# XiYe20/VPTR

Measured on AMD Instinct MI355X. Metric: predicted frames/sec (train step) NAR KTH 10->10 @64x64, higher is better.
Workload: dtype bf16x3 (split-bf16 MFMA, fp32 accumulate/storage); 1 GPU; K64: KTH 64x64x1 10->10, VPTREnc/Dec(528, Tanh, reflect) + VPTRFormerNAR(4 enc + 8 dec, d=528, 8 heads, ws 4, dropout 0.10), single_iter of train_NAR.py, random-init weights; per_gpu_batch=16, global_batch=16, frames_per_clip=10, parallelism=dp1, launch=hipGraph, dec_weight_grads=True, frozen_encoder_convs=winograd F(4x4,3x3), 36 strided-batch P16 products per convolution

## Files before the change

### vptr_amd/csrc/gemm_p16.hip

```cpp
#include "gemm_shared.h"

#include <atomic>

typedef __attribute__((ext_vector_type(4))) short s16x4;
typedef __attribute__((ext_vector_type(8))) short s16x8;

constexpr int P16_STAGE = 40 * 1024;

#define P16_GLDS(laddr, gptr) \
  asm volatile("s_mov_b32 m0, %0\n\tglobal_load_lds_dwordx4 %1, off" ::"s"(__builtin_amdgcn_readfirstlane(laddr)), "v"(gptr) : "memory")

__global__ __launch_bounds__(256) void to_p16_kernel(const float* __restrict__ x, unsigned char* __restrict__ out, int64_t n4) {
  for (int64_t i = (int64_t)blockIdx.x * 256 + threadIdx.x; i < n4; i += (int64_t)gridDim.x * 256) {
    const float4 v = reinterpret_cast<const float4*>(x)[i];
    vptr_p16_store4(out, i * 4, v);
  }
}
extern "C" int vptr_to_p16(const float* x, void* out, int64_t rows, int C, vptr_stream_t stream) {
  VPTR_CHECK(x && out && rows > 0 && C > 0 && C % 16 == 0, "to_p16: C must be a positive multiple of 16 (got %d)", C);
  VPTR_CHECK(((reinterpret_cast<uintptr_t>(x) | reinterpret_cast<uintptr_t>(out)) & 15) == 0, "to_p16: pointers must be 16-byte aligned");
  const int64_t n4 = rows * C / 4;
  to_p16_kernel<<<(unsigned)hmin64((n4 + 255) / 256, 16384), 256, 0, (hipStream_t)stream>>>(x, reinterpret_cast<unsigned char*>(out), n4);
  VPTR_LAUNCH_CHECK();
  return 0;
}

__global__ __launch_bounds__(256) void weight_planes_kernel(const vptr_wplane_entry* __restrict__ tab, const int* __restrict__ tile_start,
                                                            int count) {
  __shared__ float tile[32][33];
  const int b = blockIdx.x;
  int lo = 0, hi = count - 1;
  while (lo < hi) {
    const int mid = (lo + hi + 1) >> 1;
    if (tile_start[mid] <= b) lo = mid;
    else hi = mid - 1;
  }
  const vptr_wplane_entry e = tab[lo];
  const int t = b - tile_start[lo], tk = (e.K + 31) >> 5;
  const int n0 = (t / tk) * 32, k0 = (t % tk) * 32;
  const int r = threadIdx.x >> 3, c = (threadIdx.x & 7) * 4;
  float4 v = make_float4(0.f, 0.f, 0.f, 0.f);
  const bool ok = n0 + r < e.N && k0 + c < e.K;
  if (ok) {
    v = *reinterpret_cast<const float4*>(e.W + (int64_t)(n0 + r) * e.ldw + k0 + c);
    vptr_p16_store4(reinterpret_cast<unsigned char*>(e.Wp), (int64_t)(n0 + r) * e.K + k0 + c, v);
  }
  tile[r][c] = v.x; tile[r][c + 1] = v.y; tile[r][c + 2] = v.z; tile[r][c + 3] = v.w;
  __syncthreads();
  if (k0 + r < e.K && n0 + c < e.N) {
    const float4 w = make_float4(tile[c][r], tile[c + 1][r], tile[c + 2][r], tile[c + 3][r]);
    vptr_p16_store4(reinterpret_cast<unsigned char*>(e.WT), (int64_t)(k0 + r) * e.N + n0 + c, w);
  }
}
extern "C" int vptr_weight_planes(const vptr_wplane_entry* table_dev, const int* tile_start_dev, int count, int total_tiles,
                                  vptr_stream_t stream) {
  VPTR_CHECK(table_dev && tile_start_dev && count > 0 && total_tiles > 0, "weight_planes: bad arguments");
  weight_planes_kernel<<<total_tiles, 256, 0, (hipStream_t)stream>>>(table_dev, tile_start_dev, count);
  VPTR_LAUNCH_CHECK();
  return 0;
}

constexpr int P16_NLOAD = 4;
constexpr int P16_LONE_THREADS = GNT + 64 * P16_NLOAD;
constexpr int p16_vmcnt(const int n) { return 0x0f70 | (n & 15) | ((n >> 4) << 14); }
#define P16_GLDS_NOP(laddr, gptr) \
  asm volatile("s_mov_b32 m0, %0\n\ts_nop 0\n\tglobal_load_lds_dwordx4 %1, off" ::"s"(laddr), "v"(gptr) : "memory")

template <int EPI, int NST>
__global__ __launch_bounds__(NST == 4 ? P16_LONE_THREADS : GNT, NST == 4 ? 3 : 4) void vptr_gemm_p16_kernel(const vptr_gemm_desc p) {
  static_assert(NST == 2 || NST == 4, "two stages (two workgroups per CU) or four (one)");
  constexpr int NFN = 11, BN = 176;
  extern __shared__ __attribute__((aligned(1024))) unsigned char p16_smem[];
  const int tid = threadIdx.x, lane = tid & 63, wave = tid >> 6;
  const int wm = wave & 3, wn = wave >> 2, lr = lane & 15, lq = lane >> 4;
  const int tiles_n = (p.N + BN - 1) / BN;
  const int tiles = tiles_n * ((p.M + GBM - 1) / GBM);
  const int lg = xcd_logical_block();
  const int grp = lg / tiles, tile = lg - grp * tiles;
  const Member mb = member_of(p, p.batch > 1 ? grp : 0);
  const int m0 = (tile / tiles_n) * GBM, n0 = (tile % tiles_n) * BN;
  const int nk = (p.K + 31) >> 5;
  const bool ktail = (p.K & 16) != 0;
  const int nseg = p.ksegs > 1 ? p.ksegs : 1;
  const int64_t pa = p.lda * 4, pb = p.ldb * 4;
  const unsigned char* Ab = reinterpret_cast<const unsigned char*>(mb.A);
  const unsigned char* Bb = reinterpret_cast<const unsigned char*>(mb.B);
  const int64_t sA1 = nseg > 1 ? (p.A_x1 - p.A) * 4 : 0, sA2 = nseg > 2 ? (p.A_x2 - p.A) * 4 : 0;
  const int64_t sB1 = nseg > 1 ? (p.B_x1 - p.B) * 4 : 0, sB2 = nseg > 2 ? (p.B_x2 - p.B) * 4 : 0;

  if (NST == 4 && __builtin_amdgcn_readfirstlane(wave) >= GNT / 64) {
    const int lw = __builtin_amdgcn_readfirstlane(wave) - GNT / 64, pch = lane & 7, nkt = nk * nseg;
    constexpr int NP = 40 / P16_NLOAD, NPA = 16 / P16_NLOAD;
    const unsigned char* src[NP];
#pragma unroll
    for (int i = 0; i < NP; ++i) {
      const int u = lw + P16_NLOAD * i;
      const int prow = (i < NPA ? u : u - 16) * 8 + (lane >> 3);
      const int c = pch ^ ((prow >> 1) & 7);
      src[i] = i < NPA ? Ab + (int64_t)min(m0 + prow, p.M - 1) * pa + c * 16 : Bb + (int64_t)min(n0 + prow, p.N - 1) * pb + c * 16;
    }
    const int tadj = (pch ^ (((lane >> 4) + 4 * lw) & 7)) >= 4 ? -64 : 0;
    auto issue = [&](const int kt, const int stage) {
      const int sg = (int)(kt >= nk) + (int)(kt >= 2 * nk);
      const int kk = kt - sg * nk;
      const int64_t off = (int64_t)kk * 128 + ((ktail && kk == nk - 1) ? tadj : 0);
      int64_t oa = (sg == 0 ? (int64_t)0 : (sg == 1 ? sA1 : sA2)) + off, ob = (sg == 0 ? (int64_t)0 : (sg == 1 ? sB1 : sB2)) + off;
      asm volatile("" : "+v"(oa), "+v"(ob));
#pragma unroll
      for (int i = 0; i < NP; ++i) P16_GLDS_NOP((uint32_t)(stage * P16_STAGE + (lw + P16_NLOAD * i) * 1024), src[i] + (i < NPA ? oa : ob));
    };
    issue(0, 0);
    if (nkt > 1) issue(1, 1);
    if (nkt > 2) issue(2, 2);
    int sn = 3;
    for (int kt = 0; kt < nkt; ++kt) {
      if (kt + 2 < nkt) __builtin_amdgcn_s_waitcnt(p16_vmcnt(2 * NP));
      else if (kt + 1 < nkt) __builtin_amdgcn_s_waitcnt(p16_vmcnt(NP));
      else __builtin_amdgcn_s_waitcnt(p16_vmcnt(0));
      __syncthreads();
      if (kt + 3 < nkt) issue(kt + 3, sn);
      sn = (sn + 1) & 3;
    }
    return;
  }

  const unsigned char* srcA[2];
  const unsigned char* srcB[3];
  int tadj;
  {
    const int pch = lane & 7;
#pragma unroll
    for (int i = 0; i < 2; ++i) {
      const int prow = (wave + 8 * i) * 8 + (lane >> 3);
      const int c = pch ^ ((prow >> 1) & 7);
      srcA[i] = Ab + (int64_t)min(m0 + prow, p.M - 1) * pa + c * 16;
    }
#pragma unroll
    for (int i = 0; i < 3; ++i) {
      const int prow = (wave + 8 * i) * 8 + (lane >> 3);
      const int c = pch ^ ((prow >> 1) & 7);
      srcB[i] = Bb + (int64_t)min(n0 + prow, p.N - 1) * pb + c * 16;
    }
    const int c = pch ^ (((lane >> 4) + 4 * wave) & 7);
    tadj = c >= 4 ? -64 : 0;
  }
  auto issue1 = [&](const int kt, const int stage, const int i) {
    const int sg = (int)(kt >= nk) + (int)(kt >= 2 * nk);
    const int kk = kt - sg * nk;
    const int64_t off = (int64_t)kk * 128 + ((ktail && kk == nk - 1) ? tadj : 0);
    if (i < 2) P16_GLDS((uint32_t)(stage * P16_STAGE + (wave + 8 * i) * 1024), srcA[i] + ((sg == 0 ? (int64_t)0 : (sg == 1 ? sA1 : sA2)) + off));
    else P16_GLDS((uint32_t)(stage * P16_STAGE + 16384 + (wave + 8 * (i - 2)) * 1024), srcB[i - 2] + ((sg == 0 ? (int64_t)0 : (sg == 1 ? sB1 : sB2)) + off));
  };
  auto issue = [&](const int kt, const int stage) {
#pragma unroll
    for (int i = 0; i < 5; ++i) issue1(kt, stage, i);
  };

  f32x4 acc[2][6];
#pragma unroll
  for (int mi = 0; mi < 2; ++mi)
#pragma unroll
    for (int ni = 0; ni < 6; ++ni) acc[mi][ni] = (f32x4){0.f, 0.f, 0.f, 0.f};
  int offAh[2], offBh[6];
  const int ch = (lq >> 1) * 4 + (lq & 1);
#pragma unroll
  for (int mi = 0; mi < 2; ++mi) {
    const int r = wm * 32 + mi * 16 + lr, f = (r >> 1) & 7;
    offAh[mi] = r * 128 + ((ch ^ f) << 4);
  }
#pragma unroll
  for (int ni = 0; ni < 6; ++ni) {
    const int r = (wn * 6 + ni) * 16 + lr, f = (r >> 1) & 7;
    offBh[ni] = 16384 + r * 128 + ((ch ^ f) << 4);
  }
  const int nkt = nk * nseg;
  if (NST == 2) issue(0, 0);
  for (int kt = 0; kt < nkt; ++kt) {
    if (NST == 2) __builtin_amdgcn_s_waitcnt(0x0f70);
    __syncthreads();
    if (NST == 2 && kt + 1 < nkt) issue(kt + 1, (kt + 1) & 1);
    const unsigned char* st = p16_smem + (kt & (NST - 1)) * P16_STAGE;
    bf16x8 ah[2], al[2];
#pragma unroll
    for (int mi = 0; mi < 2; ++mi) {
      ah[mi] = *reinterpret_cast<const bf16x8*>(st + offAh[mi]);
      al[mi] = *reinterpret_cast<const bf16x8*>(st + (offAh[mi] ^ 32));
    }
    if (ktail) {
      const int sg = (int)(kt >= nk) + (int)(kt >= 2 * nk);
      if (kt - sg * nk == nk - 1 && lq >= 2) {
#pragma unroll
        for (int mi = 0; mi < 2; ++mi) {
          ah[mi] = (bf16x8){0, 0, 0, 0, 0, 0, 0, 0};
          al[mi] = (bf16x8){0, 0, 0, 0, 0, 0, 0, 0};
        }
      }
    }
    bf16x8 bh[2], bl[2];
    bh[0] = *reinterpret_cast<const bf16x8*>(st + offBh[0]);
    bl[0] = *reinterpret_cast<const bf16x8*>(st + (offBh[0] ^ 32));
#pragma unroll
    for (int ni = 0; ni < 6; ++ni) {
      if (ni == 5 && wn == 1) break;
      if (ni + 1 < 6 && !(ni + 1 == 5 && wn == 1)) {
        bh[(ni + 1) & 1] = *reinterpret_cast<const bf16x8*>(st + offBh[ni + 1]);
        bl[(ni + 1) & 1] = *reinterpret_cast<const bf16x8*>(st + (offBh[ni + 1] ^ 32));
      }
      __builtin_amdgcn_sched_barrier(0);
#pragma unroll
      for (int mi = 0; mi < 2; ++mi) {
        acc[mi][ni] = __builtin_amdgcn_mfma_f32_16x16x32_bf16(al[mi], bh[ni & 1], acc[mi][ni], 0, 0, 0);
        acc[mi][ni] = __builtin_amdgcn_mfma_f32_16x16x32_bf16(ah[mi], bl[ni & 1], acc[mi][ni], 0, 0, 0);
        acc[mi][ni] = __builtin_amdgcn_mfma_f32_16x16x32_bf16(ah[mi], bh[ni & 1], acc[mi][ni], 0, 0, 0);
      }
      __builtin_amdgcn_sched_barrier(0);
    }
  }
  constexpr bool LEAN = EPI != 0;
  if (LEAN) {
    __syncthreads();
    gemm_epilogue_rows_halves_batched<NFN, EPI>(p, mb, acc, reinterpret_cast<float*>(p16_smem), m0, n0, wm, wn, lr, lq, tid, true, false);
  } else if (NST == 4 && !p.atomic && epi_vec_ok(p)) {
    __syncthreads();
    gemm_epilogue_rows_halves_batched<NFN, 0>(p, mb, acc, reinterpret_cast<float*>(p16_smem), m0, n0, wm, wn, lr, lq, tid, true, false);
  } else if (!p.atomic && epi_vec_ok(p)) {
    __syncthreads();
    gemm_epilogue_rows_halves<NFN>(p, mb, acc, reinterpret_cast<float*>(p16_smem), m0, n0, wm, wn, lr, lq, tid, true, false);
  } else {
    gemm_epilogue_serial<NFN>(p, mb, acc, m0, n0, wm, wn, lr, lq, true, p.atomic != 0);
  }
}

__device__ __forceinline__ bf16x8 p16_tr_frag(const unsigned char* st, const int off, const int rb0) {
  const s16x4 a = __builtin_amdgcn_ds_read_tr16_b64_v4i16((__attribute__((address_space(3))) s16x4*)(st + off + rb0));
  const s16x4 b = __builtin_amdgcn_ds_read_tr16_b64_v4i16((__attribute__((address_space(3))) s16x4*)(st + off + (128 - rb0)));
  const s16x8 c = __builtin_shufflevector(a, b, 0, 1, 2, 3, 4, 5, 6, 7);
  return __builtin_bit_cast(bf16x8, c);
}

struct WgSync {
  int* cnt;
  int base;
  int n;
  bool live;
};

template <int SYNC, int MI>
__device__ __forceinline__ void wgrad_p16_tile(const vptr_gemm_desc& p, const int tile, unsigned char* p16_smem, WgSync& sy) {
  constexpr int NW = 8, BN = 176, WM = NW / 2, TR = 16 * MI * WM;
  constexpr int PA = TR / 8 / NW, PB = 24 / NW;
  constexpr int AREG = TR * 128, STG = AREG + 24 * 1024;
  const int NG = p.M, KX = p.N, T = p.K;
  const int tiles_n = (KX + BN - 1) / BN;
  const int m0 = (tile / tiles_n) * TR, n0 = (tile % tiles_n) * BN;
  const int tid = threadIdx.x, lane = tid & 63, wave = tid >> 6;
  const int wm = wave % WM, wn = wave / WM, lr = lane & 15, lq = lane >> 4;
  const int nk = (T + 31) >> 5;
  const int64_t pg = p.lda * 4, px = p.ldb * 4;
  const unsigned char* Gb = reinterpret_cast<const unsigned char*>(p.A);
  const unsigned char* Xb = reinterpret_cast<const unsigned char*>(p.B);

  int colA[PA], colB[PB], trow[PA + PB];
  {
    const int ms = lane >> 4, half = lane & 1, t = (lane & 15) >> 1;
#pragma unroll
    for (int i = 0; i < PA; ++i) {
      const int u = wave + NW * i;
      const int gran = min((m0 >> 4) + (u >> 2) * 2 + (ms >> 1), (NG >> 4) - 1);
      colA[i] = gran * 64 + (ms & 1) * 32 + half * 16;
      trow[i] = (u & 3) * 8 + t;
    }
#pragma unroll
    for (int i = 0; i < PB; ++i) {
      const int v = wave + NW * i;
      const int gran = min((n0 >> 4) + (v >> 2) * 2 + (ms >> 1), (KX >> 4) - 1);
      colB[i] = gran * 64 + (ms & 1) * 32 + half * 16;
      trow[PA + i] = (v & 3) * 8 + t;
    }
  }
  auto issue = [&](const int kt, const int stage) {
    const int t0 = kt * 32;
#pragma unroll
    for (int i = 0; i < PA; ++i)
      P16_GLDS((uint32_t)(stage * STG + (wave + NW * i) * 1024), Gb + (int64_t)min(t0 + trow[i], T - 1) * pg + colA[i]);
#pragma unroll
    for (int i = 0; i < PB; ++i)
      P16_GLDS((uint32_t)(stage * STG + AREG + (wave + NW * i) * 1024), Xb + (int64_t)min(t0 + trow[PA + i], T - 1) * px + colB[i]);
  };

  f32x4 acc[MI][6];
#pragma unroll
  for (int mi = 0; mi < MI; ++mi)
#pragma unroll
    for (int ni = 0; ni < 6; ++ni) acc[mi][ni] = (f32x4){0.f, 0.f, 0.f, 0.f};
  const int lane_off = lq * 1024 + (lr >> 2) * 32 + (lr & 3) * 8;
  const int rb0 = (lq & 1) * 128;
  int offA[MI], offB[6];
#pragma unroll
  for (int mi = 0; mi < MI; ++mi) {
    const int f = wm * MI + mi;
    offA[mi] = (f >> 1) * 4096 + (f & 1) * 512 + lane_off;
  }
#pragma unroll
  for (int ni = 0; ni < 6; ++ni) {
    const int f = wn * 6 + ni;
    offB[ni] = AREG + (f >> 1) * 4096 + (f & 1) * 512 + lane_off;
  }
  const bool flip = p.d_transposed != 0;
  const bool want_rowsum = !flip && p.a_rowsum != nullptr && n0 == 0 && wn == 1;
  const int f0 = (NG - m0 + 15) >> 4;
  const bool colsum_wave = flip && p.a_rowsum != nullptr && f0 < TR / 16 && wm == f0 / MI;
  const int cmi = f0 - wm * MI;
  const __bf16 one = (__bf16)1.0f, zero = (__bf16)0.0f;
  const bf16x8 ones = {one, one, one, one, one, one, one, one};
  const bf16x8 zeros = {zero, zero, zero, zero, zero, zero, zero, zero};
  const bool ttail = (T & 31) != 0;
  const bool rows_live = m0 + wm * (16 * MI) < NG;

  issue(0, 0);
  for (int kt = 0; kt < nk; ++kt) {
    if (SYNC > 0 && kt > 0 && (kt & (SYNC / 2 - 1)) == 0 && threadIdx.x == 0) {
      const int ph = kt & (SYNC - 1);
      if (ph == 0) __hip_atomic_fetch_add(sy.cnt, 1, __ATOMIC_RELAXED, __HIP_MEMORY_SCOPE_AGENT);
      else if (kt > SYNC && sy.live) {
        const int target = sy.base + (kt / SYNC) * sy.n;
        int spins = 0;
        while (__hip_atomic_load(sy.cnt, __ATOMIC_RELAXED, __HIP_MEMORY_SCOPE_AGENT) < target) {
          if (++spins > 3000) {
            sy.live = false;
            __hip_atomic_fetch_add(sy.cnt + 48, 1, __ATOMIC_RELAXED, __HIP_MEMORY_SCOPE_AGENT);
            break;
          }
          __builtin_amdgcn_s_sleep(8);
        }
      }
    }
    __builtin_amdgcn_s_waitcnt(0x0f70);
    __syncthreads();
    if (kt + 1 < nk) issue(kt + 1, (kt + 1) & 1);
    if (!rows_live && !colsum_wave) continue;
    const unsigned char* st = p16_smem + (kt & 1) * STG;
    bf16x8 ah[MI], al[MI];
#pragma unroll
    for (int mi = 0; mi < MI; ++mi) {
      ah[mi] = p16_tr_frag(st, offA[mi], rb0);
      al[mi] = p16_tr_frag(st, offA[mi] + 256, rb0);
    }
    if (colsum_wave) {
#pragma unroll
      for (int mi = 0; mi < MI; ++mi)
        if (mi == cmi) { ah[mi] = ones; al[mi] = zeros; }
    }
    if (ttail && kt == nk - 1) {
      const int tv = T - kt * 32;
#pragma unroll
      for (int e = 0; e < 8; ++e) {
        const int tok = 8 * lq + 4 * ((e >> 2) ^ (lq & 1)) + (e & 3);
        if (tok >= tv) {
#pragma unroll
          for (int mi = 0; mi < MI; ++mi) { ah[mi][e] = zero; al[mi][e] = zero; }
        }
      }
    }
    bf16x8 bh[2], bl[2];
    bh[0] = p16_tr_frag(st, offB[0], rb0);
    bl[0] = p16_tr_frag(st, offB[0] + 256, rb0);
#pragma unroll
    for (int ni = 0; ni < 6; ++ni) {
      if (ni == 5 && wn == 1 && !want_rowsum) break;
      if (ni + 1 < 6) {
        if (ni + 1 == 5 && wn == 1) {
          bh[(ni + 1) & 1] = ones;
          bl[(ni + 1) & 1] = zeros;
        } else {
          bh[(ni + 1) & 1] = p16_tr_frag(st, offB[ni + 1], rb0);
          bl[(ni + 1) & 1] = p16_tr_frag(st, offB[ni + 1] + 256, rb0);
        }
      }
      __builtin_amdgcn_sched_barrier(0);
#pragma unroll
      for (int mi = 0; mi < MI; ++mi) {
        acc[mi][ni] = __builtin_amdgcn_mfma_f32_16x16x32_bf16(al[mi], bh[ni & 1], acc[mi][ni], 0, 0, 0);
        acc[mi][ni] = __builtin_amdgcn_mfma_f32_16x16x32_bf16(ah[mi], bl[ni & 1], acc[mi][ni], 0, 0, 0);
        acc[mi][ni] = __builtin_amdgcn_mfma_f32_16x16x32_bf16(ah[mi], bh[ni & 1], acc[mi][ni], 0, 0, 0);
      }
      __builtin_amdgcn_sched_barrier(0);
    }
  }
  const float alpha = p.alpha;
#pragma unroll
  for (int ni = 0; ni < 6; ++ni) {
    const int nf = wn * 6 + ni, col = n0 + nf * 16 + lr;
    if (nf < 11 && col < KX) {
#pragma unroll
      for (int mi = 0; mi < MI; ++mi)
#pragma unroll
        for (int r = 0; r < 4; ++r) {
          const int row = m0 + (wm * MI + mi) * 16 + lq * 4 + r;
          if (row < NG) {
            float* dst = flip ? p.D + (int64_t)col * p.ldd + row : p.D + (int64_t)row * p.ldd + col;
            if (p.atomic) unsafeAtomicAdd(dst, acc[mi][ni][r] * alpha);
            else *dst = acc[mi][ni][r] * alpha;
          }
        }
    }
  }
  if (colsum_wave && lq == 0) {
#pragma unroll
    for (int ni = 0; ni < 6; ++ni) {
      const int nf = wn * 6 + ni, col = n0 + nf * 16 + lr;
      if (nf < 11 && col < KX) {
        float cs = 0.f;
#pragma unroll
        for (int mi = 0; mi < MI; ++mi)
          if (mi == cmi) cs = acc[mi][ni][0];
        unsafeAtomicAdd(p.a_rowsum + col, cs * alpha);
      }
    }
  }
  if (want_rowsum && lr == 0) {
#pragma unroll
    for (int mi = 0; mi < MI; ++mi)
#pragma unroll
      for (int r = 0; r < 4; ++r) {
        const int row = m0 + (wm * MI + mi) * 16 + lq * 4 + r;
        if (row < NG) unsafeAtomicAdd(p.a_rowsum + row, acc[mi][5][r] * alpha);
      }
  }
}


template <int NSTAGE, int TAG = 0, int NW = 8, int MI = 16 / NW>
__global__ __launch_bounds__(64 * NW, MI == 2 ? 4 : 2) void vptr_wgrad_p16_kernel(const vptr_gemm_desc* __restrict__ descs, const int* __restrict__ tile_start,
                                                                            const int count) {
  static_assert(NSTAGE == 2 && NW == 8, "two stages, eight waves");
  extern __shared__ __attribute__((aligned(1024))) unsigned char p16_smem[];
  const int lg = xcd_logical_block();
  int lo = 0, hi = count - 1;
  while (lo < hi) {
    const int mid = (lo + hi + 1) >> 1;
    if (tile_start[mid] <= lg) lo = mid;
    else hi = mid - 1;
  }
  WgSync none = {nullptr, 0, 0, false};
  wgrad_p16_tile<0, MI>(descs[lo], lg - tile_start[lo], p16_smem, none);
}

__device__ int g_wgrad_sync_ws[8 * 64];
template <int S, int NW = 8, int MI = 16 / NW, int NST = 2>
__global__ __launch_bounds__(64 * NW, MI == 2 ? 4 : 2) void vptr_wgrad_p16_sync_kernel(const vptr_gemm_desc* __restrict__ descs, const int* __restrict__ tile_start,
                                                                const int count, const int total_tiles) {
  static_assert(NST == 2 && NW == 8, "two stages, eight waves");
  extern __shared__ __attribute__((aligned(1024))) unsigned char p16_smem[];
  int* const ws = g_wgrad_sync_ws;
  const int xcd = blockIdx.x & 7, slot = blockIdx.x >> 3, slots = gridDim.x >> 3;
  const int xq = total_tiles >> 3, xr = total_tiles & 7;
  const int first = xcd * xq + min(xcd, xr), mine = xq + (xcd < xr ? 1 : 0);
  const int nk = (descs[0].K + 31) >> 5;
  const int per_tile = (nk - 1) / S;
  WgSync sy = {ws + xcd * 64, 0, 0, true};
  for (int r = 0; r * slots + slot < mine; ++r) {
    const int lg = first + r * slots + slot;
    int lo = 0, hi = count - 1;
    while (lo < hi) {
      const int mid = (lo + hi + 1) >> 1;
      if (tile_start[mid] <= lg) lo = mid;
      else hi = mid - 1;
    }
    sy.base = r * slots * per_tile;
    sy.n = min(slots, mine - r * slots);
    if (r > 0) __syncthreads();
    wgrad_p16_tile<S, MI>(descs[lo], lg - tile_start[lo], p16_smem, sy);
  }
  if (threadIdx.x == 0) {
    int* done = ws + xcd * 64 + 32;
    if (__hip_atomic_fetch_add(done, 1, __ATOMIC_RELAXED, __HIP_MEMORY_SCOPE_AGENT) == slots - 1) {
      __hip_atomic_store(ws + xcd * 64, 0, __ATOMIC_RELAXED, __HIP_MEMORY_SCOPE_AGENT);
      __hip_atomic_store(done, 0, __ATOMIC_RELAXED, __HIP_MEMORY_SCOPE_AGENT);
    }
  }
}

__global__ void wgrad_sync_stats_kernel(int* __restrict__ out) {
  if (threadIdx.x < 8) out[threadIdx.x] = g_wgrad_sync_ws[threadIdx.x * 64 + 48];
}
extern "C" int vptr_wgrad_sync_stats(int* out_dev, vptr_stream_t stream) {
  VPTR_CHECK(out_dev != nullptr, "wgrad_sync_stats: null output");
  wgrad_sync_stats_kernel<<<1, 64, 0, (hipStream_t)stream>>>(out_dev);
  VPTR_LAUNCH_CHECK();
  return 0;
}

static int vptr_cu_count() {
  static int n = -1;
  if (n < 0) {
    int dev = 0, v = 0;
    if (hipGetDevice(&dev) == hipSuccess && hipDeviceGetAttribute(&v, hipDeviceAttributeMultiprocessorCount, dev) == hipSuccess) n = v;
    else n = 0;
  }
  return n;
}

template <int EPI>
static bool p16_reserve_lds() {
  return hipFuncSetAttribute(reinterpret_cast<const void*>(&vptr_gemm_p16_kernel<EPI, 2>), hipFuncAttributeMaxDynamicSharedMemorySize, 2 * P16_STAGE) == hipSuccess &&
         hipFuncSetAttribute(reinterpret_cast<const void*>(&vptr_gemm_p16_kernel<EPI, 4>), hipFuncAttributeMaxDynamicSharedMemorySize, 4 * P16_STAGE) == hipSuccess;
}

template <int EPI>
static void p16_launch(const vptr_gemm_desc& d, const int tiles, const bool lone, hipStream_t st) {
  if (lone) vptr_gemm_p16_kernel<EPI, 4><<<tiles, P16_LONE_THREADS, 4 * P16_STAGE, st>>>(d);
  else vptr_gemm_p16_kernel<EPI, 2><<<tiles, GNT, 2 * P16_STAGE, st>>>(d);
}

int vptr_gemm_p16_launch(vptr_gemm_desc& d, hipStream_t st) {
  VPTR_CHECK(d.a_mode == VPTR_A_P16 && d.b_mode == VPTR_B_P16, "vptr_gemm(p16): both operands must be P16 (a_mode %d, b_mode %d)", d.a_mode, d.b_mode);
  VPTR_CHECK(d.K % 16 == 0 && d.lda % 16 == 0 && d.ldb % 16 == 0, "vptr_gemm(p16): K, lda, ldb must be multiples of 16 (K %d)", d.K);
  VPTR_CHECK(d.split_k <= 1 && d.precision == 3 && !d.a_rowsum && !d.D_planes, "vptr_gemm(p16): split_k = 1, precision 3, no a_rowsum / D_planes");
  if (d.alpha == 0.f) d.alpha = 1.f;
  if (d.batch < 1) d.batch = 1;
  if (d.ksegs < 1) d.ksegs = 1;
  const bool strided = d.batch_stride_d != 0;
  if (strided)
    VPTR_CHECK(d.ksegs == 1 && d.batch <= 4096 && !d.Dpre && !d.residual && !d.atomic && !d.batch_accum && !d.frame_stats && !d.act_grad_src && !d.rowscale &&
                   !d.colscale && d.dropout_p == 0.f && d.act == VPTR_ACT_NONE && !d.act_after &&
                   ((d.batch_stride_a | d.batch_stride_b | d.batch_stride_d) & 15) == 0 && d.batch_stride_a >= 0 && d.batch_stride_b >= 0 && d.batch_stride_d > 0,
               "vptr_gemm(p16): a strided batch takes bias / alpha only and strides that are non-negative multiples of 16");
// ... 116 lines not shown
```

### vptr_amd/csrc/gemm_shared.h

```cpp
#pragma once
#include "common.h"

#define GBM 128
#define GBK 32
#define GLP 32
#define GNT 512

typedef __attribute__((ext_vector_type(2))) __bf16 bf16x2;
typedef __attribute__((ext_vector_type(2))) float f32x2;

__device__ __forceinline__ float4 mask4(const float4 v, const unsigned m) {
  float4 o;
  o.x = __uint_as_float(__float_as_uint(v.x) & m);
  o.y = __uint_as_float(__float_as_uint(v.y) & m);
  o.z = __uint_as_float(__float_as_uint(v.z) & m);
  o.w = __uint_as_float(__float_as_uint(v.w) & m);
  return o;
}

__device__ __forceinline__ uint32_t pk_bf16(const float a, const float b) {
  const f32x2 f = {a, b};
  const bf16x2 h = __builtin_convertvector(f, bf16x2);
  return *reinterpret_cast<const uint32_t*>(&h);
}
// ... 97 lines not shown
      }
    }
  } else {
#pragma unroll
    for (int ni = g0; ni < g0 + GW && ni < NFW; ++ni) {
#pragma unroll
      for (int mi = 0; mi < 2; ++mi) {
#pragma unroll
        for (int r = 0; r < 4; ++r) {
          const int row = row_base + mi * 16 + r;
          if (colok[ni] && row < p.M) {
            float v = (acc[mi][ni][r] * cs[ni] + bs[ni]) * mb.alpha;
            if (p.Dpre) p.Dpre[(int64_t)row * p.ldd + col[ni]] = v;
            v = vptr_act(v, p.act) * rsv[mi][r];
            if (p.dropout_p > 0.f) v *= vptr_drop_scale(seed, p.site, (uint64_t)row * (uint64_t)p.N + col[ni], p.dropout_p);
            v += res[ni - g0][mi][r];
            if (p.act_after) v = v > 0.f ? v : 0.f;
            float* dst = mb.D + epi_drow(p, row) * p.ldd + col[ni];
            if (use_atomic) unsafeAtomicAdd(dst, v);
            else *dst = v;
          }
        }
      }
    }
  }
  }
}


template <int NFN>
constexpr int epi_lds_bytes() { return GBM * (16 * NFN + 4) * (int)sizeof(float); }

__device__ __forceinline__ bool epi_vec_ok(const vptr_gemm_desc& p) {
  uintptr_t bits = reinterpret_cast<uintptr_t>(p.D) | reinterpret_cast<uintptr_t>(p.Dpre) | reinterpret_cast<uintptr_t>(p.residual) |
                   reinterpret_cast<uintptr_t>(p.bias) | reinterpret_cast<uintptr_t>(p.colscale);
  if (p.batch > 1 && p.batch_stride_d == 0) bits |= reinterpret_cast<uintptr_t>(p.D_x1) | reinterpret_cast<uintptr_t>(p.D_x2) | reinterpret_cast<uintptr_t>(p.bias_x1) |
                           reinterpret_cast<uintptr_t>(p.bias_x2);
  return ((bits & 15) == 0) && ((p.N & 3) == 0) && ((p.ldd & 3) == 0) && ((p.ldr & 3) == 0);
}

template <int NFN>
__device__ __forceinline__ void gemm_epilogue_rows(const vptr_gemm_desc& p, const Member& mb, f32x4 (&acc)[2][(NFN + 1) / 2], float* sE, const int m0,
                                                   const int n0, const int wm, const int wn, const int lr, const int lq, const int tid,
                                                   const bool first_split, const bool use_atomic) {
  constexpr int NFW = (NFN + 1) / 2, BN = 16 * NFN, PITCH = BN + 4, C4 = BN / 4;
#pragma unroll
  for (int ni = 0; ni < NFW; ++ni) {
    const int nf = wn * NFW + ni;
    if (nf < NFN) {
#pragma unroll
      for (int mi = 0; mi < 2; ++mi)
#pragma unroll
        for (int r = 0; r < 4; ++r) sE[(wm * 32 + mi * 16 + lq * 4 + r) * PITCH + nf * 16 + lr] = acc[mi][ni][r];
    }
  }
  __syncthreads();
  const bool has_res = p.residual && first_split;
  const bool has_bias = mb.bias && first_split;
  f32x4 res[NFN], bs[NFN];
  float rsv[NFN];
#pragma unroll
  for (int it = 0; it < NFN; ++it) {
    const int piece = it * GNT + tid;
    const int rl = piece / C4;
    const int row = m0 + rl, col = n0 + (piece - rl * C4) * 4;
    const bool ok = row < p.M && col < p.N;
    bs[it] = res[it] = (f32x4){0.f, 0.f, 0.f, 0.f};
    rsv[it] = 1.f;
    if (has_bias && ok) bs[it] = *reinterpret_cast<const f32x4*>(mb.bias + col);
    if (p.rowscale && ok) rsv[it] = p.rowscale[(row / p.rs_div) % p.rs_mod];
    if (has_res && ok) res[it] = *reinterpret_cast<const f32x4*>(p.residual + (int64_t)row * p.ldr + col);
  }
  uint64_t seed = 0;
  if (p.dropout_p > 0.f) seed = *p.seed_dev;
  const bool plain = !p.colscale && !p.Dpre && p.act == VPTR_ACT_NONE && !p.rowscale && p.dropout_p == 0.f && !p.act_after &&
                     mb.alpha == 1.f;
#pragma unroll
  for (int it = 0; it < NFN; ++it) {
    const int piece = it * GNT + tid;
    const int rl = piece / C4;
    const int row = m0 + rl, col = n0 + (piece - rl * C4) * 4;
    if (row < p.M && col < p.N) {
      f32x4 v = *reinterpret_cast<const f32x4*>(&sE[rl * PITCH + (piece - rl * C4) * 4]);
      if (plain) {
        v = v + bs[it] + res[it];
      } else {
        if (p.colscale) v = v * *reinterpret_cast<const f32x4*>(p.colscale + col);
        v = (v + bs[it]) * mb.alpha;
        if (p.Dpre) *reinterpret_cast<f32x4*>(p.Dpre + (int64_t)row * p.ldd + col) = v;
#pragma unroll
        for (int e = 0; e < 4; ++e) {
          float t = vptr_act(v[e], p.act) * rsv[it];
          if (p.dropout_p > 0.f) t *= vptr_drop_scale(seed, p.site, (uint64_t)row * (uint64_t)p.N + col + e, p.dropout_p);
          t += res[it][e];
          if (p.act_after) t = t > 0.f ? t : 0.f;
          v[e] = t;
        }
      }
      float* dst = mb.D + epi_drow(p, row) * p.ldd + col;
      if (use_atomic) {
#pragma unroll
        for (int e = 0; e < 4; ++e) unsafeAtomicAdd(dst + e, v[e]);
      } else {
        *reinterpret_cast<f32x4*>(dst) = v;
      }
    }
  }
  __syncthreads();
}


template <int NFN>
constexpr int epi_half_lds_bytes() { return (GBM / 2) * (16 * NFN + 4) * (int)sizeof(float); }

template <int NFN>
__device__ __forceinline__ void gemm_epilogue_rows_halves(const vptr_gemm_desc& p, const Member& mb, f32x4 (&acc)[2][(NFN + 1) / 2], float* sE,
                                                          const int m0, const int n0, const int wm, const int wn, const int lr, const int lq,
                                                          const int tid, const bool first_split, const bool use_atomic) {
  constexpr int NFW = (NFN + 1) / 2, BN = 16 * NFN, PITCH = BN + 4, C4 = BN / 4, HR = GBM / 2, NPIECE = HR * C4;
  const bool has_res = p.residual && first_split;
  const bool has_bias = mb.bias && first_split;
  uint64_t seed = 0;
  if (p.dropout_p > 0.f) seed = *p.seed_dev;
#pragma unroll
  for (int h = 0; h < 2; ++h) {
    if ((wm >> 1) == h) {
#pragma unroll
      for (int ni = 0; ni < NFW; ++ni) {
        const int nf = wn * NFW + ni;
        if (nf < NFN) {
#pragma unroll
          for (int mi = 0; mi < 2; ++mi)
#pragma unroll
            for (int r = 0; r < 4; ++r) sE[((wm & 1) * 32 + mi * 16 + lq * 4 + r) * PITCH + nf * 16 + lr] = acc[mi][ni][r];
        }
      }
    }
    __syncthreads();
#pragma unroll
    for (int it = 0; it < (NPIECE + GNT - 1) / GNT; ++it) {
      const int piece = it * GNT + tid;
      const int rl = piece / C4;
      const int row = m0 + h * HR + rl, col = n0 + (piece - rl * C4) * 4;
      if (piece < NPIECE && row < p.M && col < p.N) {
        f32x4 v = *reinterpret_cast<const f32x4*>(&sE[rl * PITCH + (piece - rl * C4) * 4]);
        if (p.colscale) v = v * *reinterpret_cast<const f32x4*>(p.colscale + col);
        if (has_bias) v = v + *reinterpret_cast<const f32x4*>(mb.bias + col);
        v = v * mb.alpha;
        if (p.Dpre) *reinterpret_cast<f32x4*>(p.Dpre + (int64_t)row * p.ldd + col) = v;
        f32x4 res = {0.f, 0.f, 0.f, 0.f};
        if (has_res) res = *reinterpret_cast<const f32x4*>(p.residual + (int64_t)row * p.ldr + col);
        const float rs = p.rowscale ? p.rowscale[(row / p.rs_div) % p.rs_mod] : 1.f;
#pragma unroll
        for (int e = 0; e < 4; ++e) {
          float t = vptr_act(v[e], p.act) * rs;
          if (p.dropout_p > 0.f) t *= vptr_drop_scale(seed, p.site, (uint64_t)row * (uint64_t)p.N + col + e, p.dropout_p);
          t += res[e];
          if (p.act_after) t = t > 0.f ? t : 0.f;
          v[e] = t;
        }
        if (p.D_planes) {
          uint32_t hi[2], lo[2];
          split2(v[0], v[1], hi[0], lo[0]);
          split2(v[2], v[3], hi[1], lo[1]);
          __bf16* o = reinterpret_cast<__bf16*>(p.D_planes) + ((int64_t)row * ((p.N + 31) >> 5) + (col >> 5)) * 64 + (col & 31);
          *reinterpret_cast<uint2*>(o) = make_uint2(hi[0], hi[1]);
          *reinterpret_cast<uint2*>(o + 32) = make_uint2(lo[0], lo[1]);
        }
        if (mb.D) {
          float* dst = mb.D + epi_drow(p, row) * p.ldd + col;
          if (p.d_p16) {
            vptr_p16_store4(reinterpret_cast<unsigned char*>(mb.D), (int64_t)row * p.ldd + col, make_float4(v[0], v[1], v[2], v[3]));
          } else if (use_atomic) {
#pragma unroll
            for (int e = 0; e < 4; ++e) unsafeAtomicAdd(dst + e, v[e]);
          } else {
            *reinterpret_cast<f32x4*>(dst) = v;
          }
        }
      }
    }
    if (h == 0) __syncthreads();
  }
}


template <int NFN, int EPI>
__device__ __forceinline__ void gemm_epilogue_rows_halves_batched(const vptr_gemm_desc& p, const Member& mb, f32x4 (&acc)[2][(NFN + 1) / 2], float* sE,
                                                          const int m0, const int n0, const int wm, const int wn, const int lr, const int lq,
                                                          const int tid, const bool first_split, const bool use_atomic_in) {
  constexpr int NFW = (NFN + 1) / 2, BN = 16 * NFN, PITCH = BN + 4, C4 = BN / 4, HR = GBM / 2, NPIECE = HR * C4;
  constexpr bool LEAN = EPI != 0, GRAD = EPI == 2;
  const bool has_res = !GRAD && mb.res && first_split;
  const bool has_bias = !GRAD && mb.bias && first_split;
  const bool use_atomic = !LEAN && use_atomic_in;
  const float* const colscale = LEAN ? nullptr : p.colscale;
  float* const Dpre = (LEAN && EPI != 4) ? nullptr : p.Dpre;
  const float* const rowscale = (LEAN && EPI != 3) ? nullptr : p.rowscale;
  const auto D_planes = LEAN ? decltype(p.D_planes)(nullptr) : p.D_planes;
  const int act = (EPI == 1 || EPI == 3) ? VPTR_ACT_NONE : p.act;
  const float dropout_p = EPI == 1 ? 0.f : p.dropout_p;
  const bool act_after = !LEAN && p.act_after;
  uint64_t seed = 0;
  if (dropout_p > 0.f) seed = *p.seed_dev;
  constexpr int NIT = (NPIECE + GNT - 1) / GNT;
  float bs[NFW], cs[NFW];
#pragma unroll
  for (int ni = 0; ni < NFW; ++ni) {
    const int nf = wn * NFW + ni, col = n0 + nf * 16 + lr;
    const bool ok = (nf < NFN) & (col < p.N);
    bs[ni] = (has_bias && ok) ? mb.bias[col] : 0.f;
    cs[ni] = (colscale && ok) ? colscale[col] : 1.f;
  }
#pragma unroll
  for (int h = 0; h < 2; ++h) {
    f32x4 res[NIT];
    float rsv[NIT];
    float ssum = 0.f, ssq = 0.f;
#pragma unroll
    for (int it = 0; it < NIT; ++it) {
      const int piece = it * GNT + tid;
      const int rl = piece / C4;
      const int row = m0 + h * HR + rl, col = n0 + (piece - rl * C4) * 4;
      const bool ok = piece < NPIECE && row < p.M && col < p.N;
      res[it] = (f32x4){0.f, 0.f, 0.f, 0.f};
      if (has_res && ok) res[it] = *reinterpret_cast<const f32x4*>(mb.res + (int64_t)row * mb.ldr + col);
      if (GRAD && ok) res[it] = *reinterpret_cast<const f32x4*>(p.act_grad_src + (int64_t)row * p.ldd + col);
      rsv[it] = (rowscale && ok) ? rowscale[(row / p.rs_div) % p.rs_mod] : 1.f;
    }
    if ((wm >> 1) == h) {
#pragma unroll
      for (int ni = 0; ni < NFW; ++ni) {
        const int nf = wn * NFW + ni;
        if (nf < NFN) {
#pragma unroll
          for (int mi = 0; mi < 2; ++mi)
#pragma unroll
            for (int r = 0; r < 4; ++r)
              sE[((wm & 1) * 32 + mi * 16 + lq * 4 + r) * PITCH + nf * 16 + lr] = (acc[mi][ni][r] * cs[ni] + bs[ni]) * mb.alpha;
        }
      }
    }
    __syncthreads();
#pragma unroll
    for (int it = 0; it < NIT; ++it) {
      const int piece = it * GNT + tid;
      const int rl = piece / C4;
      const int row = m0 + h * HR + rl, col = n0 + (piece - rl * C4) * 4;
      if (piece < NPIECE && row < p.M && col < p.N) {
        f32x4 v = *reinterpret_cast<const f32x4*>(&sE[rl * PITCH + (piece - rl * C4) * 4]);
        if (Dpre) *reinterpret_cast<f32x4*>(Dpre + (int64_t)row * p.ldd + col) = v;
        const float rs = rsv[it];
#pragma unroll
        for (int e = 0; e < 4; ++e) {
          float t = GRAD ? v[e] * vptr_act_grad(res[it][e], act) : vptr_act(v[e], act) * rs;
          if (dropout_p > 0.f) t *= vptr_drop_scale(seed, p.site, (uint64_t)row * (uint64_t)p.N + col + e, dropout_p);
          t += GRAD ? 0.f : res[it][e];
          if (act_after) t = t > 0.f ? t : 0.f;
          v[e] = t;
        }
        if (!GRAD && p.frame_stats) {
          ssum += (v[0] + v[1]) + (v[2] + v[3]);
          ssq += (v[0] * v[0] + v[1] * v[1]) + (v[2] * v[2] + v[3] * v[3]);
        }
        if (D_planes) {
          uint32_t hi[2], lo[2];
          split2(v[0], v[1], hi[0], lo[0]);
          split2(v[2], v[3], hi[1], lo[1]);
          __bf16* o = reinterpret_cast<__bf16*>(D_planes) + ((int64_t)row * ((p.N + 31) >> 5) + (col >> 5)) * 64 + (col & 31);
          *reinterpret_cast<uint2*>(o) = make_uint2(hi[0], hi[1]);
          *reinterpret_cast<uint2*>(o + 32) = make_uint2(lo[0], lo[1]);
        }
        if (mb.D) {
          float* dst = mb.D + epi_drow(p, row) * p.ldd + col;
          if (p.d_p16) {
            vptr_p16_store4(reinterpret_cast<unsigned char*>(mb.D), (int64_t)row * p.ldd + col, make_float4(v[0], v[1], v[2], v[3]));
          } else if (use_atomic) {
#pragma unroll
            for (int e = 0; e < 4; ++e) unsafeAtomicAdd(dst + e, v[e]);
          } else {
            *reinterpret_cast<f32x4*>(dst) = v;
          }
        }
      }
    }
    if (!GRAD && p.frame_stats) {
      const float S = wave_sum(ssum), Q = wave_sum(ssq);
      float* red = sE + HR * PITCH;
      if ((tid & 63) == 0) { red[2 * (tid >> 6)] = S; red[2 * (tid >> 6) + 1] = Q; }
      __syncthreads();
      if (tid == 0 && m0 + h * HR < p.M) {
        float s8 = 0.f, q8 = 0.f;
#pragma unroll
        for (int w = 0; w < GNT / 64; ++w) { s8 += red[2 * w]; q8 += red[2 * w + 1]; }
        const int fr = (m0 + h * HR) / p.frame_rows;
        unsafeAtomicAdd(p.frame_stats + VPTR_FRAME_STATS_STRIDE * fr, s8);
        unsafeAtomicAdd(p.frame_stats + VPTR_FRAME_STATS_STRIDE * fr + 1, q8);
      }
    }
    if (h == 0) __syncthreads();
  }
}


template <int NFN>
__device__ __forceinline__ void gemm_epilogue_serial(const vptr_gemm_desc& p, const Member& mb, f32x4 (&acc)[2][(NFN + 1) / 2], const int m0, const int n0,
                                              const int wm, const int wn, const int lr, const int lq, const bool first_split,
                                              const bool use_atomic) {
  constexpr int NFW = (NFN + 1) / 2;
  const bool plain = !p.colscale && !p.Dpre && p.act == VPTR_ACT_NONE && !p.rowscale && p.dropout_p == 0.f && !p.act_after &&
                     mb.alpha == 1.f;
  const int row_base = m0 + wm * 32 + lq * 4;
  if (plain) {
#pragma unroll
    for (int ni = 0; ni < NFW; ++ni) {
      const int nf = wn * NFW + ni;
      const int col = n0 + nf * 16 + lr;
      const bool colok = (nf < NFN) & (col < p.N);
      const float bs = (mb.bias && first_split && colok) ? mb.bias[col] : 0.f;
#pragma unroll
      for (int mi = 0; mi < 2; ++mi) {
#pragma unroll
        for (int r = 0; r < 4; ++r) {
          const int row = row_base + mi * 16 + r;
          if (colok && row < p.M) {
            float v = acc[mi][ni][r] + bs;
            if (p.residual && first_split) v += p.residual[(int64_t)row * p.ldr + col];
            float* dst = mb.D + epi_drow(p, row) * p.ldd + col;
            if (use_atomic) unsafeAtomicAdd(dst, v);
            else *dst = v;
          }
        }
      }
    }
  } else {
    uint64_t seed = 0;
    if (p.dropout_p > 0.f) seed = *p.seed_dev;
#pragma unroll
    for (int ni = 0; ni < NFW; ++ni) {
      const int nf = wn * NFW + ni;
      const int col = n0 + nf * 16 + lr;
      const bool colok = (nf < NFN) & (col < p.N);
      const float bs = (mb.bias && first_split && colok) ? mb.bias[col] : 0.f;
      const float cs = (p.colscale && colok) ? p.colscale[col] : 1.f;
#pragma unroll
      for (int mi = 0; mi < 2; ++mi) {
#pragma unroll
        for (int r = 0; r < 4; ++r) {
          const int row = row_base + mi * 16 + r;
          if (colok && row < p.M) {
            float v = (acc[mi][ni][r] * cs + bs) * mb.alpha;
            if (p.Dpre) p.Dpre[(int64_t)row * p.ldd + col] = v;
            v = vptr_act(v, p.act);
            if (p.rowscale) v *= p.rowscale[(row / p.rs_div) % p.rs_mod];
            if (p.dropout_p > 0.f) v = v * vptr_drop_scale(seed, p.site, (uint64_t)row * (uint64_t)p.N + col, p.dropout_p) + 0.f;
            if (p.residual && first_split) v += p.residual[(int64_t)row * p.ldr + col];
            if (p.act_after) v = v > 0.f ? v : 0.f;
            float* dst = mb.D + epi_drow(p, row) * p.ldd + col;
            if (use_atomic) unsafeAtomicAdd(dst, v);
            else *dst = v;
          }
        }
      }
    }
  }
}


__device__ __forceinline__ int xcd_logical_block() {
  const int nblk = gridDim.x, xq = nblk >> 3, xr = nblk & 7, xcd = blockIdx.x & 7;
  return xcd * xq + min(xcd, xr) + (blockIdx.x >> 3);
}


int vptr_gemm_p16_launch(vptr_gemm_desc& d, hipStream_t st);
int vptr_wgrad_p16_launch(const vptr_gemm_desc* proto, const vptr_gemm_desc* descs_dev, const int* tile_start_dev, int count, int total_tiles,
                          hipStream_t st);
```

Baseline: 3752 frames/s.

## Prefetch epilogue operands during K-loop tail and let loader waves join epilogue

In the four-stage P16 GEMM, the epilogue's bias, colscale, residual and rowscale loads for the first half-tile are issued a few K-steps before the main loop ends, so their latency hides behind the last MFMA iterations. The dedicated loader waves, which used to exit once their DMA issues finished, now also prefetch their share of half-0 operands and then take part in the epilogue, which is strided over all threads. This spreads the epilogue across more threads and overlaps its global loads with compute. The cost is higher register pressure from the held operands and more complex vmcnt and barrier accounting, including a barrier count that must match between loader and compute waves.

```diff
diff --git a/vptr_amd/csrc/gemm_p16.hip b/vptr_amd/csrc/gemm_p16.hip
--- a/vptr_amd/csrc/gemm_p16.hip
+++ b/vptr_amd/csrc/gemm_p16.hip
@@ -65,6 +65,19 @@
 constexpr int p16_vmcnt(const int n) { return 0x0f70 | (n & 15) | ((n >> 4) << 14); }
 #define P16_GLDS_NOP(laddr, gptr) \
   asm volatile("s_mov_b32 m0, %0\n\ts_nop 0\n\tglobal_load_lds_dwordx4 %1, off" ::"s"(laddr), "v"(gptr) : "memory")
+template <int DMA, int PER>
+__device__ __forceinline__ void p16_wait_tail(const int kinds) {
+  if (kinds == 0) __builtin_amdgcn_s_waitcnt(p16_vmcnt(DMA));
+  else if (kinds == 1) __builtin_amdgcn_s_waitcnt(p16_vmcnt(DMA + PER));
+  else __builtin_amdgcn_s_waitcnt(p16_vmcnt(DMA + 2 * PER));
+}
+
+template <int NFN, int EPI, int NTH>
+__device__ __forceinline__ void p16_request_half0(const vptr_gemm_desc& p, const Member& mb, const int m0, const int n0, const int wn, const int lr, const int tid,
+                                                  EpiHalf0<NFN, NTH>& pre) {
+  gemm_epilogue_request_cols<NFN, EPI>(p, mb, n0, wn, lr, true, pre.bs, pre.cs);
+  gemm_epilogue_request_half<NFN, EPI, NTH, false, epi_half_nit<NFN, NTH>()>(p, mb, m0, n0, tid, 0, true, pre.res, pre.rsv);
+}
 
 template <int EPI, int NST>
 __global__ __launch_bounds__(NST == 4 ? P16_LONE_THREADS : GNT, NST == 4 ? 3 : 4) void vptr_gemm_p16_kernel(const vptr_gemm_desc p) {
@@ -88,9 +101,12 @@
   const int64_t sA1 = nseg > 1 ? (p.A_x1 - p.A) * 4 : 0, sA2 = nseg > 2 ? (p.A_x2 - p.A) * 4 : 0;
   const int64_t sB1 = nseg > 1 ? (p.B_x1 - p.B) * 4 : 0, sB2 = nseg > 2 ? (p.B_x2 - p.B) * 4 : 0;
 
+  constexpr bool LEAN = EPI != 0;
+  constexpr int ETH = NST == 4 ? P16_LONE_THREADS : GNT;
   if (NST == 4 && __builtin_amdgcn_readfirstlane(wave) >= GNT / 64) {
     const int lw = __builtin_amdgcn_readfirstlane(wave) - GNT / 64, pch = lane & 7, nkt = nk * nseg;
     constexpr int NP = 40 / P16_NLOAD, NPA = 16 / P16_NLOAD;
+    EpiHalf0<NFN, ETH> pre;
     const unsigned char* src[NP];
 #pragma unroll
     for (int i = 0; i < NP; ++i) {
@@ -113,14 +129,33 @@
     if (nkt > 1) issue(1, 1);
     if (nkt > 2) issue(2, 2);
     int sn = 3;
-    for (int kt = 0; kt < nkt; ++kt) {
-      if (kt + 2 < nkt) __builtin_amdgcn_s_waitcnt(p16_vmcnt(2 * NP));
-      else if (kt + 1 < nkt) __builtin_amdgcn_s_waitcnt(p16_vmcnt(NP));
-      else __builtin_amdgcn_s_waitcnt(p16_vmcnt(0));
+    for (int kt = 0; kt + 3 < nkt; ++kt) {
+      __builtin_amdgcn_s_waitcnt(p16_vmcnt(2 * NP));
       __syncthreads();
-      if (kt + 3 < nkt) issue(kt + 3, sn);
+      issue(kt + 3, sn);
       sn = (sn + 1) & 3;
     }
+    if (nkt >= 3) {
+      __builtin_amdgcn_s_waitcnt(p16_vmcnt(2 * NP));
+      __syncthreads();
+    }
+    constexpr int NPL = (64 * 44 - GNT + ETH - 1) / ETH;
+    const bool joins = LEAN || (!p.atomic && epi_vec_ok(p));
+    int kinds = 0;
+    if (joins) {
+      kinds = gemm_epilogue_half_load_kinds<EPI>(p, mb, true);
+      gemm_epilogue_request_half<NFN, EPI, ETH, true, NPL>(p, mb, m0, n0, tid, 0, true, pre.res, pre.rsv);
+    }
+    if (nkt >= 2) {
+      p16_wait_tail<NP, NPL>(kinds);
+      __syncthreads();
+    }
+    p16_wait_tail<0, NPL>(kinds);
+    __syncthreads();
+    if (!joins) return;
+    f32x4 none[2][6];
+    __syncthreads();
+    gemm_epilogue_rows_halves_lone<NFN, EPI, ETH, true>(p, mb, none, reinterpret_cast<float*>(p16_smem), m0, n0, wm, wn, lr, lq, tid, true, false, false, &pre, true);
     return;
   }
 
@@ -174,11 +209,15 @@
     offBh[ni] = 16384 + r * 128 + ((ch ^ f) << 4);
   }
   const int nkt = nk * nseg;
+  EpiHalf0<NFN, ETH> pre;
+  const bool hoist = NST == 4 && (EPI != 0 || (!p.atomic && epi_vec_ok(p)));
+  if (hoist && nkt < 3) p16_request_half0<NFN, EPI, ETH>(p, mb, m0, n0, wn, lr, tid, pre);
   if (NST == 2) issue(0, 0);
   for (int kt = 0; kt < nkt; ++kt) {
     if (NST == 2) __builtin_amdgcn_s_waitcnt(0x0f70);
     __syncthreads();
     if (NST == 2 && kt + 1 < nkt) issue(kt + 1, (kt + 1) & 1);
+    if (hoist && kt + 3 == nkt) p16_request_half0<NFN, EPI, ETH>(p, mb, m0, n0, wn, lr, tid, pre);
     const unsigned char* st = p16_smem + (kt & (NST - 1)) * P16_STAGE;
     bf16x8 ah[2], al[2];
 #pragma unroll
@@ -216,13 +255,15 @@
       __builtin_amdgcn_sched_barrier(0);
     }
   }
-  constexpr bool LEAN = EPI != 0;
   if (LEAN) {
     __syncthreads();
-    gemm_epilogue_rows_halves_batched<NFN, EPI>(p, mb, acc, reinterpret_cast<float*>(p16_smem), m0, n0, wm, wn, lr, lq, tid, true, false);
+    if (NST == 4)
+      gemm_epilogue_rows_halves_lone<NFN, EPI, ETH, true>(p, mb, acc, reinterpret_cast<float*>(p16_smem), m0, n0, wm, wn, lr, lq, tid, true, false, true, &pre, hoist);
+    else
+      gemm_epilogue_rows_halves_batched<NFN, EPI>(p, mb, acc, reinterpret_cast<float*>(p16_smem), m0, n0, wm, wn, lr, lq, tid, true, false);
   } else if (NST == 4 && !p.atomic && epi_vec_ok(p)) {
     __syncthreads();
-    gemm_epilogue_rows_halves_batched<NFN, 0>(p, mb, acc, reinterpret_cast<float*>(p16_smem), m0, n0, wm, wn, lr, lq, tid, true, false);
+    gemm_epilogue_rows_halves_lone<NFN, 0, ETH, true>(p, mb, acc, reinterpret_cast<float*>(p16_smem), m0, n0, wm, wn, lr, lq, tid, true, false, true, &pre, hoist);
   } else if (!p.atomic && epi_vec_ok(p)) {
     __syncthreads();
     gemm_epilogue_rows_halves<NFN>(p, mb, acc, reinterpret_cast<float*>(p16_smem), m0, n0, wm, wn, lr, lq, tid, true, false);
diff --git a/vptr_amd/csrc/gemm_shared.h b/vptr_amd/csrc/gemm_shared.h
--- a/vptr_amd/csrc/gemm_shared.h
+++ b/vptr_amd/csrc/gemm_shared.h
@@ -423,6 +423,183 @@
   }
 }
 
+template <int NFN, int NTH>
+constexpr int epi_half_nit() { return ((GBM / 2) * (16 * NFN / 4) + NTH - 1) / NTH; }
+
+template <int NFN, int NTH>
+struct EpiHalf0 {
+  float bs[(NFN + 1) / 2], cs[(NFN + 1) / 2];
+  f32x4 res[epi_half_nit<NFN, NTH>()];
+  float rsv[epi_half_nit<NFN, NTH>()];
+};
+
+template <int EPI>
+__device__ __forceinline__ int gemm_epilogue_half_load_kinds(const vptr_gemm_desc& p, const Member& mb, const bool first_split) {
+  constexpr bool LEAN = EPI != 0, GRAD = EPI == 2;
+  const bool has_res = !GRAD && mb.res && first_split;
+  const float* const rowscale = (LEAN && EPI != 3) ? nullptr : p.rowscale;
+  return (int)(has_res || GRAD) + (int)(rowscale != nullptr);
+}
+
+template <int NFN, int EPI>
+__device__ __forceinline__ void gemm_epilogue_request_cols(const vptr_gemm_desc& p, const Member& mb, const int n0, const int wn, const int lr,
+                                                           const bool first_split, float (&bs)[(NFN + 1) / 2], float (&cs)[(NFN + 1) / 2]) {
+  constexpr int NFW = (NFN + 1) / 2;
+  constexpr bool LEAN = EPI != 0, GRAD = EPI == 2;
+  const bool has_bias = !GRAD && mb.bias && first_split;
+  const float* const colscale = LEAN ? nullptr : p.colscale;
+#pragma unroll
+  for (int ni = 0; ni < NFW; ++ni) {
+    const int nf = wn * NFW + ni, col = n0 + nf * 16 + lr;
+    const bool ok = (nf < NFN) & (col < p.N);
+    bs[ni] = (has_bias && ok) ? mb.bias[col] : 0.f;
+    cs[ni] = (colscale && ok) ? colscale[col] : 1.f;
+  }
+}
+
+template <int NFN, int EPI, int NTH, bool CLAMP, int CNT>
+__device__ __forceinline__ void gemm_epilogue_request_half(const vptr_gemm_desc& p, const Member& mb, const int m0, const int n0, const int tid, const int h,
+                                                           const bool first_split, f32x4 (&res)[epi_half_nit<NFN, NTH>()],
+                                                           float (&rsv)[epi_half_nit<NFN, NTH>()]) {
+  constexpr int BN = 16 * NFN, C4 = BN / 4, HR = GBM / 2, NPIECE = HR * C4, NIT = epi_half_nit<NFN, NTH>();
+  constexpr bool LEAN = EPI != 0, GRAD = EPI == 2;
+  const bool has_res = !GRAD && mb.res && first_split;
+  const float* const rowscale = (LEAN && EPI != 3) ? nullptr : p.rowscale;
+#pragma unroll
+  for (int it = 0; it < NIT; ++it) {
+    if (it >= CNT) {
+      res[it] = (f32x4){0.f, 0.f, 0.f, 0.f};
+      rsv[it] = 1.f;
+    } else if (CLAMP) {
+      const int piece = min(it * NTH + tid, NPIECE - 1);
+      const int rl = piece / C4;
+      const int row = min(m0 + h * HR + rl, p.M - 1), col = min(n0 + (piece - rl * C4) * 4, p.N - 4);
+      res[it] = (f32x4){0.f, 0.f, 0.f, 0.f};
+      rsv[it] = 1.f;
+      if (has_res) res[it] = *reinterpret_cast<const f32x4*>(mb.res + (int64_t)row * mb.ldr + col);
+      if (GRAD) res[it] = *reinterpret_cast<const f32x4*>(p.act_grad_src + (int64_t)row * p.ldd + col);
+      if (rowscale) rsv[it] = rowscale[(row / p.rs_div) % p.rs_mod];
+    } else {
+      const int piece = it * NTH + tid;
+      const int rl = piece / C4;
+      const int row = m0 + h * HR + rl, col = n0 + (piece - rl * C4) * 4;
+      const bool ok = piece < NPIECE && row < p.M && col < p.N;
+      res[it] = (f32x4){0.f, 0.f, 0.f, 0.f};
+      if (has_res && ok) res[it] = *reinterpret_cast<const f32x4*>(mb.res + (int64_t)row * mb.ldr + col);
+      if (GRAD && ok) res[it] = *reinterpret_cast<const f32x4*>(p.act_grad_src + (int64_t)row * p.ldd + col);
+      rsv[it] = (rowscale && ok) ? rowscale[(row / p.rs_div) % p.rs_mod] : 1.f;
+    }
+  }
+}
+
+template <int NFN, int EPI, int NTH, bool PRE>
+__device__ __forceinline__ void gemm_epilogue_rows_halves_lone(const vptr_gemm_desc& p, const Member& mb, f32x4 (&acc)[2][(NFN + 1) / 2], float* sE,
+                                                          const int m0, const int n0, const int wm, const int wn, const int lr, const int lq,
+                                                          const int tid, const bool first_split, const bool use_atomic_in,
+                                                          const bool spills, const EpiHalf0<NFN, NTH>* pre, const bool pre_ok) {
+  constexpr int NFW = (NFN + 1) / 2, BN = 16 * NFN, PITCH = BN + 4, C4 = BN / 4, HR = GBM / 2, NPIECE = HR * C4;
+  constexpr bool LEAN = EPI != 0, GRAD = EPI == 2;
+  const bool use_atomic = !LEAN && use_atomic_in;
+  float* const Dpre = (LEAN && EPI != 4) ? nullptr : p.Dpre;
+  const auto D_planes = LEAN ? decltype(p.D_planes)(nullptr) : p.D_planes;
+  const int act = (EPI == 1 || EPI == 3) ? VPTR_ACT_NONE : p.act;
+  const float dropout_p = EPI == 1 ? 0.f : p.dropout_p;
+  const bool act_after = !LEAN && p.act_after;
+  uint64_t seed = 0;
+  if (dropout_p > 0.f) seed = *p.seed_dev;
+  constexpr int NIT = epi_half_nit<NFN, NTH>();
+  float bs[NFW], cs[NFW];
+  if (PRE && pre_ok) {
+#pragma unroll
+    for (int ni = 0; ni < NFW; ++ni) { bs[ni] = pre->bs[ni]; cs[ni] = pre->cs[ni]; }
+  } else {
+    gemm_epilogue_request_cols<NFN, EPI>(p, mb, n0, wn, lr, first_split, bs, cs);
+  }
+#pragma unroll
+  for (int h = 0; h < 2; ++h) {
+    f32x4 res[NIT];
+    float rsv[NIT];
+    float ssum = 0.f, ssq = 0.f;
+    if (PRE && h == 0 && pre_ok) {
+#pragma unroll
+      for (int it = 0; it < NIT; ++it) { res[it] = pre->res[it]; rsv[it] = pre->rsv[it]; }
+    } else {
+      gemm_epilogue_request_half<NFN, EPI, NTH, false, NIT>(p, mb, m0, n0, tid, h, first_split, res, rsv);
+    }
+    if (spills && (wm >> 1) == h) {
+#pragma unroll
+      for (int ni = 0; ni < NFW; ++ni) {
+        const int nf = wn * NFW + ni;
+        if (nf < NFN) {
+#pragma unroll
+          for (int mi = 0; mi < 2; ++mi)
+#pragma unroll
+            for (int r = 0; r < 4; ++r)
+              sE[((wm & 1) * 32 + mi * 16 + lq * 4 + r) * PITCH + nf * 16 + lr] = (acc[mi][ni][r] * cs[ni] + bs[ni]) * mb.alpha;
+        }
+      }
+    }
+    __syncthreads();
+#pragma unroll
+    for (int it = 0; it < NIT; ++it) {
+      const int piece = it * NTH + tid;
+      const int rl = piece / C4;
+      const int row = m0 + h * HR + rl, col = n0 + (piece - rl * C4) * 4;
+      if (piece < NPIECE && row < p.M && col < p.N) {
+        f32x4 v = *reinterpret_cast<const f32x4*>(&sE[rl * PITCH + (piece - rl * C4) * 4]);
+        if (Dpre) *reinterpret_cast<f32x4*>(Dpre + (int64_t)row * p.ldd + col) = v;
+        const float rs = rsv[it];
+#pragma unroll
+        for (int e = 0; e < 4; ++e) {
+          float t = GRAD ? v[e] * vptr_act_grad(res[it][e], act) : vptr_act(v[e], act) * rs;
+          if (dropout_p > 0.f) t *= vptr_drop_scale(seed, p.site, (uint64_t)row * (uint64_t)p.N + col + e, dropout_p);
+          t += GRAD ? 0.f : res[it][e];
+          if (act_after) t = t > 0.f ? t : 0.f;
+          v[e] = t;
+        }
+        if (!GRAD && p.frame_stats) {
+          ssum += (v[0] + v[1]) + (v[2] + v[3]);
+          ssq += (v[0] * v[0] + v[1] * v[1]) + (v[2] * v[2] + v[3] * v[3]);
+        }
+        if (D_planes) {
+          uint32_t hi[2], lo[2];
+          split2(v[0], v[1], hi[0], lo[0]);
+          split2(v[2], v[3], hi[1], lo[1]);
+          __bf16* o = reinterpret_cast<__bf16*>(D_planes) + ((int64_t)row * ((p.N + 31) >> 5) + (col >> 5)) * 64 + (col & 31);
+          *reinterpret_cast<uint2*>(o) = make_uint2(hi[0], hi[1]);
+          *reinterpret_cast<uint2*>(o + 32) = make_uint2(lo[0], lo[1]);
+        }
+        if (mb.D) {
+          float* dst = mb.D + epi_drow(p, row) * p.ldd + col;
+          if (p.d_p16) {
+            vptr_p16_store4(reinterpret_cast<unsigned char*>(mb.D), (int64_t)row * p.ldd + col, make_float4(v[0], v[1], v[2], v[3]));
+          } else if (use_atomic) {
+#pragma unroll
+            for (int e = 0; e < 4; ++e) unsafeAtomicAdd(dst + e, v[e]);
+          } else {
+            *reinterpret_cast<f32x4*>(dst) = v;
+          }
+        }
+      }
+    }
+    if (!GRAD && p.frame_stats) {
+      const float S = wave_sum(ssum), Q = wave_sum(ssq);
+      float* red = sE + HR * PITCH;
+      if ((tid & 63) == 0) { red[2 * (tid >> 6)] = S; red[2 * (tid >> 6) + 1] = Q; }
+      __syncthreads();
+      if (tid == 0 && m0 + h * HR < p.M) {
+        float s8 = 0.f, q8 = 0.f;
+#pragma unroll
+        for (int w = 0; w < NTH / 64; ++w) { s8 += red[2 * w]; q8 += red[2 * w + 1]; }
+        const int fr = (m0 + h * HR) / p.frame_rows;
+        unsafeAtomicAdd(p.frame_stats + VPTR_FRAME_STATS_STRIDE * fr, s8);
+        unsafeAtomicAdd(p.frame_stats + VPTR_FRAME_STATS_STRIDE * fr + 1, q8);
+      }
+    }
+    if (h == 0) __syncthreads();
+  }
+}
+
 
 template <int NFN>
 __device__ __forceinline__ void gemm_epilogue_serial(const vptr_gemm_desc& p, const Member& mb, f32x4 (&acc)[2][(NFN + 1) / 2], const int m0, const int n0,
```

Result: no change. 3758 frames/s (median of 2 runs) (+0.1%).
